# bramtoula/multi_robot_SLAM_separators

Measured on AMD Instinct MI355X. Metric: candidate keyframe-pair verifications/sec (NetVLAD NN + ORB match + RANSAC) @1/2/4/8 GPU, higher is better.
Workload: dtype u8+f16+f32+f64

## Files before the change

### multi_robot_slam_separators_amd/csrc/k_match.hip

```cpp
#include "sf_internal.hpp"
#include "sf_match_device.hpp"
#include <type_traits>

namespace {

__device__ __forceinline__ uint32_t bcnt_acc(uint32_t x, uint32_t acc) {
  uint32_t r;
  asm("v_bcnt_u32_b32 %0, %1, %2" : "=v"(r) : "v"(x), "v"(acc));
  return r;
}

template <int W, int NQ>
__device__ __forceinline__ void knn2_scan(const uint32_t* __restrict__ dF, int Kf, const uint32_t (&q)[NQ][W],
                                          uint32_t (&k1)[NQ], uint32_t (&k2)[NQ]) {
#pragma unroll 4
  for (int f = 0; f < Kf; ++f) {
    const uint32_t* r = dF + (size_t)f * W;
    uint32_t x[W];
#pragma unroll
    for (int c = 0; c < W; ++c) x[c] = r[c];
#pragma unroll
    for (int j = 0; j < NQ; ++j) {
      uint32_t d = 0;
#pragma unroll
// ... 448 lines not shown
        constexpr int JP = NTL - 1;
        float t;
        const int jp = j == 0 ? JP : j - 1;
        mf_pipe_half1(acc0, A4[0], A4[1], A4[2], A4[3], B4[j][0], B4[j][1], c0, acc1, b[jp], s[jp], t);
        mf_pipe_half2(acc0, A4[2], A4[3], B4[j][2], B4[j][3], acc1, b[jp], s[jp], t);
        mf_pipe_half1(acc1, A4[0], A4[1], A4[2], A4[3], B4[j + 1][0], B4[j + 1][1], c0, acc0, b[j], s[j], t);
        mf_pipe_half2(acc1, A4[2], A4[3], B4[j + 1][2], B4[j + 1][3], acc0, b[j], s[j], t);
      }
    }
  }
  mf_pipe_drain(acc1, b[NTL - 1], s[NTL - 1]);
}

__device__ __forceinline__ float mf_max(float a, float b) {
  float r;
  asm("v_max_f32 %0, %1, %2" : "=v"(r) : "v"(a), "v"(b));
  return r;
}
__device__ __forceinline__ float mf_min(float a, float b) {
  float r;
  asm("v_min_f32 %0, %1, %2" : "=v"(r) : "v"(a), "v"(b));
  return r;
}
__device__ __forceinline__ float mf_max3(float a, float b, float c) {
  float r;
  asm("v_max3_f32 %0, %1, %2, %3" : "=v"(r) : "v"(a), "v"(b), "v"(c));
  return r;
}

constexpr int mf_passes(int ntl) { return ntl == 1 ? 1 : ntl / 2; }

template <int W, int NTL, bool PIPE = false>
__device__ __forceinline__ void mf_scan(const uint32_t* fromD, int Kf, const MfB<W, NTL>& B, int lane,
                                        uint32_t (&d1)[mf_passes(NTL)], uint32_t (&d2)[mf_passes(NTL)],
                                        int (&idx)[mf_passes(NTL)]) {
  constexpr int KS = W / 2;
  const int r = lane & 31, h = lane >> 5;
  uint32_t m88, c22;
  asm volatile("v_mov_b32 %0, 0x88888888" : "=v"(m88));
  asm volatile("v_mov_b32 %0, 0x22222222" : "=v"(c22));
  float cin[16], b[NTL], s[NTL];
  const float hoff = h ? 4.f * MF_FR : 0.f;
#pragma unroll
  for (int i = 0; i < 16; ++i) cin[i] = -(float)((i & 3) + 8 * (i >> 2)) * MF_FR - hoff;
#pragma unroll
  for (int j = 0; j < NTL; ++j) { b[j] = -INFINITY; s[j] = -INFINITY; }
  const int n_full = Kf >> 5;
  uint32_t raw[KS];
  load_raw<KS>(fromD + (size_t)min(r, Kf - 1) * W + KS * h, raw);
  const uint32_t* nxt = fromD + (size_t)r * W + KS * h;
  if constexpr (PIPE && W == 8 && (NTL == 2 || NTL == 4)) {
    mf_scan_tiles_pipe<NTL>(fromD, n_full, Kf & 31, B, cin, b, s, m88, c22, raw, nxt);
  } else {
    for (int mt = 0; mt < n_full; ++mt) knn2_mfma_tile<W, NTL, false>(fromD, Kf, mt, r, h, B.Bf, cin, b, s, m88, c22, raw, nxt);
    if (Kf & 31) knn2_mfma_tile<W, NTL, true>(fromD, Kf, n_full, r, h, B.Bf, cin, b, s, m88, c22, raw, nxt);
  }
  const float org = (float)(32 * (((Kf + 31) >> 5) - 1)) * MF_FR;
#pragma unroll
  for (int p = 0; p < mf_passes(NTL); ++p) {
    float mb, ms, ob, os;
    int ts;
    if constexpr (NTL == 1) {
      mb = b[0]; ms = s[0]; ts = 24 * W - 2 * (int)B.psum;
      ob = __shfl_xor(mb, 32); os = __shfl_xor(ms, 32);
    } else {
      const int j0 = 2 * p, j1 = 2 * p + 1;
      mb = h ? b[j1] : b[j0]; ms = h ? s[j1] : s[j0]; ts = 24 * W - 2 * (int)((B.psum >> (16 * p + 8 * h)) & 0xFFu);
      ob = __shfl_xor(h ? b[j0] : b[j1], 32); os = __shfl_xor(h ? s[j0] : s[j1], 32);
    }
    const float nb = mf_max(mb, ob) - org;
    const float ns = mf_max3(mf_min(mb, ob), ms, os) - org;
    const float dot1 = 2.f * ceilf(nb * 0.5f), dot2 = 2.f * ceilf(ns * 0.5f);
    idx[p] = (int)((dot1 - nb) * 2048.f);
    d1[p] = (uint32_t)((32 * W - ts - (int)dot1) >> 1);
    d2[p] = ns == -INFINITY ? 0xFFFFu : (uint32_t)((32 * W - ts - (int)dot2) >> 1);
  }
}

template <int W, int NTL, bool PIPE = false>
__device__ __forceinline__ void knn2_mfma(const uint32_t* fromD, int Kf, const uint32_t* __restrict__ dT, int Kt,
                                          const int (&tile)[NTL], int lane, uint32_t (&d1)[mf_passes(NTL)],
                                          uint32_t (&d2)[mf_passes(NTL)], int (&idx)[mf_passes(NTL)]) {
  asm volatile("" : "+v"(lane));
  MfB<W, NTL> B;
  mf_load_b<W, NTL>(dT, Kt, tile, lane, B);
  mf_scan<W, NTL, PIPE>(fromD, Kf, B, lane, d1, d2, idx);
}

template <int W>
__device__ __forceinline__ uint32_t mf_repair_d2(const uint32_t* fromD, int Kf, const uint32_t* __restrict__ q_row, int idx,
                                                 uint32_t d2) {
  if ((idx & 27) == 27) return d2;
  uint32_t q[W];
  load_raw<W>(q_row, q);
  const int base = (idx & ~31) + (idx & 4);
#pragma unroll 1
  for (int g = 0; g < 32; g += 8) {
#pragma unroll
    for (int k = 0; k < 4; ++k) {
      const int row = base + g + k;
      uint32_t x[W];
      load_raw<W>(fromD + (size_t)row * W, x);
      uint32_t d = 0;
#pragma unroll
      for (int c = 0; c < W; ++c) d = bcnt_acc(x[c] ^ q[c], d);
      const bool other = row < Kf && row != idx && (g + k) != 27;
      d2 = other ? min(d2, d) : d2;
    }
  }
  return d2;
}

__device__ __forceinline__ int mf_rank_below(unsigned long long mask) {
  return (int)__builtin_amdgcn_mbcnt_hi((uint32_t)(mask >> 32), __builtin_amdgcn_mbcnt_lo((uint32_t)mask, 0u));
}

template <int W>
__device__ __forceinline__ bool mf_repair_accept(const uint32_t* fromD, int Kf, const uint32_t* __restrict__ q_row, int idx,
                                                 uint32_t d1, uint32_t d2, float nndr, bool active) {
  bool acc = false, exact = active;
  if (nndr >= 0.f) {
    if (active) {
      uint32_t pmin = d2;
      if ((idx & 27) != 27) {
        uint32_t q[4];
        load_raw<4>(q_row, q);
        const int base = (idx & ~31) + (idx & 4);
        const uint32_t ok = ((1u << min(Kf - base, 31)) - 1u) & ~(1u << (idx - base)) & ~(1u << 27);
        uint32_t no = __builtin_amdgcn_alignbit(~ok, ~ok, 23);
#pragma unroll 1
        for (int g = 0; g < 32; g += 8) {
#pragma unroll
          for (int k = 0; k < 4; ++k) {
            uint32_t x[4];
            load_raw<4>(fromD + (size_t)(base + g + k) * W, x);
            uint32_t p = no & (512u << k);
#pragma unroll
            for (int c = 0; c < 4; ++c) p = bcnt_acc(x[c] ^ q[c], p);
            pmin = min(pmin, p);
          }
          no = __builtin_amdgcn_alignbit(no, no, 8);
        }
      }
      acc = !((float)d1 > nndr * (float)pmin);
      exact = !acc;
    }
  }
  if (__ballot(exact)) {
    if (exact) acc = !((float)d1 > nndr * (float)mf_repair_d2<W>(fromD, Kf, q_row, idx, d2));
  }
  return acc;
}

template <int W, int NQ, int NT, int MF_NTL = 2, bool MF_PIPE = false>
__device__ __forceinline__ bool match_v2_body(const StoreView& st, int pair, int sF, int sT, float nndr, int min_inliers,
                                              int est, uint32_t* out, CorrHeader& hdr_out, PassState& pass_out,
                                              int32_t* __restrict__ list, int32_t* __restrict__ counter, int* smem,
                                              unsigned long long* trace_row = nullptr) {
  constexpr int NW = NT / 64;
  const int tid = threadIdx.x;
  const int lane = tid & 63, wave = __builtin_amdgcn_readfirstlane(tid >> 6);
  const int kcap = st.kcap;
  if ((unsigned)sF >= (unsigned)st.n_slots || (unsigned)sT >= (unsigned)st.n_slots) {
    if (tid == 0) {
      CorrHeader h = {0, 0, 0, 0};
      hdr_out = h;
      write_null_pass(pass_out, 0);
    }
    return false;
  }
  const int4 mF = st.meta[sF], mT = st.meta[sT];
  const int Kf = mF.x, Kt = mT.x;
  const uint32_t* dF = st.desc + (size_t)sF * kcap * W;
  const uint32_t* dT = st.desc + (size_t)sT * kcap * W;

  uint32_t* fromD = reinterpret_cast<uint32_t*>(smem);
  int* cnt = smem + kcap * W;
  int* owner = cnt + kcap;
  int* misc = owner + kcap;

  {
    const uint4* src = reinterpret_cast<const uint4*>(dF);
    uint4* dst = reinterpret_cast<uint4*>(fromD);
    for (int i = tid; i < Kf * (W / 4); i += NT) dst[i] = src[i];
  }
  for (int i = tid; i < Kf; i += NT) cnt[i] = 0;
  if (tid < 16) misc[tid] = 0;
  __syncthreads();
  SF_TRACE_ROW_MARK(trace_row, 32);

  int rejected = 0;
  if constexpr (NQ == 0) {
    if (Kf > 0) {
      constexpr int NTL = W == 8 ? MF_NTL : 1;
      const int n_nt = (Kt + 31) >> 5;
      auto group = [&](auto g, int t0) {
        constexpr int G = decltype(g)::value, NP = mf_passes(G);
        int tl[G], f[NP];
        uint32_t a1[NP], a2[NP];
#pragma unroll
        for (int j = 0; j < G; ++j) tl[j] = t0 + j * NW;
        knn2_mfma<W, G, MF_PIPE>(fromD, Kf, dT, Kt, tl, lane, a1, a2, f);
        int t[NP];
        bool on[NP], acc[NP], redo[NP];
#pragma unroll
        for (int p = 0; p < NP; ++p) {
          t[p] = G == 1 ? tl[0] * 32 + lane : (tl[2 * p] + (lane >> 5) * NW) * 32 + (lane & 31);
          on[p] = (G > 1 || lane < 32) && t[p] < Kt;
          acc[p] = (Kf >= 2) && !((float)a1[p] > nndr * (float)a2[p]);
          redo[p] = on[p] && Kf >= 2 && (acc[p] || !(nndr >= 0.f));
        }
        if constexpr (NP == 1) {
          if (__ballot(redo[0])) {
            const bool r = mf_repair_accept<W>(fromD, Kf, dT + (size_t)t[0] * W, f[0], a1[0], a2[0], nndr, redo[0]);
            acc[0] = redo[0] ? r : acc[0];
          }
        } else {
          static_assert(NP == 2, "a group has one or two decode passes");
          const unsigned long long bal0 = __ballot(redo[0]), bal1 = __ballot(redo[1]);
          const int n0 = __popcll(bal0), n1 = __popcll(bal1);
          const bool merged = nndr >= 0.f && n0 != 0 && n1 != 0 && n0 + n1 <= 64;
          int tgt = 0;
          uint32_t m0 = 0, m1 = 0;
          bool mine = false;
          if (merged) {
            const int jf = mf_rank_below(~bal0), r1 = mf_rank_below(bal1);
            const int dest = redo[0] ? 64 - n0 + lane - jf : jf;
            const int slot = __builtin_amdgcn_ds_permute(dest << 2, lane);
            tgt = __builtin_amdgcn_ds_bpermute((redo[1] ? r1 : n1 + lane - r1) << 2, slot);
            m0 = (uint32_t)__builtin_amdgcn_ds_permute(tgt << 2, (int)((uint32_t)t[1] | ((uint32_t)f[1] << 16)));
            m1 = (uint32_t)__builtin_amdgcn_ds_permute(tgt << 2, (int)(a1[1] | (a2[1] << 16)));
            mine = !redo[0] && jf < n1;
          }
#pragma unroll 1
          for (int it = 0; it < 2; ++it) {
            bool act = it ? redo[1] : redo[0];
            int wt = it ? t[1] : t[0], wf = it ? f[1] : f[0];
            uint32_t w1 = it ? a1[1] : a1[0], w2 = it ? a2[1] : a2[0];
            if (mine) {
              act = true;
              wt = (int)(m0 & 0xFFFFu); wf = (int)(m0 >> 16);
              w1 = m1 & 0xFFFFu; w2 = m1 >> 16;
            }
            if (__ballot(act)) {
              const bool r = mf_repair_accept<W>(fromD, Kf, dT + (size_t)wt * W, wf, w1, w2, nndr, act);
              if (merged) {
                const bool back = __builtin_amdgcn_ds_bpermute(tgt << 2, (int)r) != 0;
                acc[0] = redo[0] ? r : acc[0];
                acc[1] = redo[1] ? back : acc[1];
              } else if (it) {
                acc[1] = redo[1] ? r : acc[1];
              } else {
                acc[0] = redo[0] ? r : acc[0];
              }
            }
            if (merged) break;
          }
        }
#pragma unroll
        for (int p = 0; p < NP; ++p) {
          if (on[p] && acc[p]) match_claim(cnt, owner, f[p], t[p]);
          rejected += __popcll(__ballot(on[p] && !acc[p]));
        }
      };
      for (int t0 = wave; t0 < n_nt; t0 += NW * NTL) {
        const int avail = (n_nt - t0 + NW - 1) / NW;
        if constexpr (NTL >= 4) {
          if (avail >= 3) { group(std::integral_constant<int, 4>{}, t0); continue; }
        }
        if constexpr (NTL >= 2) {
          if (avail >= 2) { group(std::integral_constant<int, 2>{}, t0); continue; }
        }
        group(std::integral_constant<int, 1>{}, t0);
      }
    }
  } else if (Kf > 0) {
    for (int base = 0; base < Kt; base += NQ * NT) {

      uint32_t q[NQ][W], d1[NQ], d2[NQ], chunk[NQ];
#pragma unroll
      for (int j = 0; j < NQ; ++j) {
        const int t = base + j * NT + tid;
        load_desc<W>(dT, t, t < Kt, q[j]);
        d1[j] = 0xFFFFu;
        d2[j] = 0xFFFFu;
        chunk[j] = 0;
      }
      const int wave_rows = Kt - base - (tid & ~63);
      const int groups = wave_rows <= 0 ? 0 : min(NQ, (wave_rows + NT - 1) / NT);
      if (groups == NQ) {
        knn2_scan_lds<W, NQ>(fromD, Kf, q, d1, d2, chunk);
      } else if (groups > 0) {
#pragma unroll
        for (int j = 0; j < NQ; ++j) {
          if (j < groups) {
            uint32_t qq[1][W], a1[1] = {0xFFFFu}, a2[1] = {0xFFFFu}, ch[1] = {0};
#pragma unroll
            for (int c = 0; c < W; ++c) qq[0][c] = q[j][c];
            knn2_scan_lds<W, 1>(fromD, Kf, qq, a1, a2, ch);
            d1[j] = a1[0]; d2[j] = a2[0]; chunk[j] = ch[0];
          }
        }
      }
#pragma unroll
      for (int j = 0; j < NQ; ++j) {
        const int t = base + j * NT + tid;
        if (t < Kt) {
          const uint32_t b1 = d1[j] & 0xFFFFu, b2 = d2[j] & 0xFFFFu;
          const bool acc = (Kf >= 2) && !((float)b1 > nndr * (float)b2);
          if (acc) {
            int f = (int)chunk[j];
            const int fend = min(f + MATCH_CH, Kf);
            for (; f < fend; ++f) {
              const uint32_t* r = fromD + (size_t)f * W;
              uint32_t d = 0;
#pragma unroll
              for (int c = 0; c < W; ++c) d += __popc(r[c] ^ q[j][c]);
              if (d == b1) break;
            }
            match_claim(cnt, owner, f, t);
          } else {
            ++rejected;
          }
        }
      }
    }
  }
  if constexpr (NQ != 0) {
    for (int off = 32; off >= 1; off >>= 1) rejected += __shfl_xor(rejected, off);
  }
  if (lane == 0 && rejected) atomicAdd(&misc[0], rejected);
  SF_TRACE_ROW_MARK(trace_row, 33);
  __syncthreads();
  SF_TRACE_ROW_MARK(trace_row, 34);

  int running = 0;
  for (int base = 0; base < Kf; base += NT) {
    const int f = base + tid;
    const bool flag = (f < Kf) && (cnt[f] == 1);
    const unsigned long long bal = __ballot(flag);
    const int before = __popcll(bal & ((1ull << lane) - 1ull));
    if (lane == 0) misc[4 + wave] = __popcll(bal);
    __syncthreads();
    int woff = 0, total = 0;
#pragma unroll
    for (int w = 0; w < NW; ++w) {
      int c = misc[4 + w];
      if (w < wave) woff += c;
      total += c;
    }
    if (flag) out[running + woff + before] = (uint32_t)f | ((uint32_t)owner[f] << 16);
    running += total;
    __syncthreads();
  }
  const int n_corr = running;
  SF_TRACE_ROW_MARK(trace_row, 35);

  const MatchGates G = match_gates(Kf, Kt, mF, mT, misc[0], n_corr, min_inliers, est);
  const bool motion = G.motion, survivor = G.survivor;
  if (motion && !survivor)
    corr_count_finite<NT>(st.xyz + (size_t)sF * kcap * 3, st.xyz + (size_t)sT * kcap * 3, out, n_corr, est == 0, &misc[2]);
  if (tid == 0) {
    CorrHeader h;
    h.n_corr = n_corr;
    h.words_from = G.words_from;
    h.words_to = G.words_to;
    h.words_to_2d = G.unique_to;
    hdr_out = h;
    write_null_pass(pass_out, (motion && !survivor) ? misc[2] : 0);
    if (survivor && list) worklist_append(list, counter, pair);
  }
  return survivor;
}

template <int W, int NQ, int NT>
__global__ void __launch_bounds__(NT)
k_match_global_v2(StoreView st, const int32_t* __restrict__ pair_from, const int32_t* __restrict__ pair_to,
                  float nndr, int min_inliers, int est, uint32_t* __restrict__ corr, CorrHeader* __restrict__ hdr,
                  PassState* __restrict__ pass, int32_t* __restrict__ list, int32_t* __restrict__ counter) {
  extern __shared__ __attribute__((aligned(16))) int smem[];
  const int pair = (int)blockIdx.x;
  match_v2_body<W, NQ, NT>(st, pair, pair_from[pair], pair_to[pair], nndr, min_inliers, est, corr + (size_t)pair * st.kcap,
                           hdr[pair], pass[pair], list, counter, smem);
}

template <int W, int NT>
__global__ void __launch_bounds__(NT, 2)
k_match_global_mf(StoreView st, const int32_t* __restrict__ pair_from, const int32_t* __restrict__ pair_to,
                  float nndr, int min_inliers, int est, uint32_t* __restrict__ corr, CorrHeader* __restrict__ hdr,
                  PassState* __restrict__ pass, int32_t* __restrict__ list, int32_t* __restrict__ counter) {
  extern __shared__ __attribute__((aligned(16))) int smem[];
  const int pair = (int)blockIdx.x;
  match_v2_body<W, 0, NT, 4>(st, pair, pair_from[pair], pair_to[pair], nndr, min_inliers, est,
                             corr + (size_t)pair * st.kcap, hdr[pair], pass[pair], list, counter, smem);
}

template <int W, int NQ, int NT>
void launch_match_v2(sf_context* c, StoreView st, const int32_t* d_from, const int32_t* d_to, int n) {
  size_t lds = sf_match_lds_bytes(st.kcap, W);
  if (const char* v = getenv("SF_MATCH_LDS_PAD")) lds += (size_t)atoi(v);
  if constexpr (NQ == 0) sf_launch_pass1(c, k_match_global_mf<W, NT>, NT, lds, st, d_from, d_to, n);
  else sf_launch_pass1(c, k_match_global_v2<W, NQ, NT>, NT, lds, st, d_from, d_to, n);
}

template <int W, int NQ, int NT, bool L2 = false>
void launch_match(sf_context* c, StoreView st, const int32_t* d_from, const int32_t* d_to, int n) {
  sf_launch_pass1(c, k_match_global<W, NQ, NT, L2>, NT, (size_t)(2 * st.kcap + 16) * sizeof(int), st, d_from, d_to, n);
}

}

int sf_launch_match_global(sf_context* c, StoreView st, const int32_t* d_from, const int32_t* d_to, int n) {
  if (n <= 0) return SF_OK;
  if (c->params.desc_type == 2) return sf_launch_match_global_u8(c, st, d_from, d_to, n);
  if (c->params.desc_type == 1) {
    sf_prof_begin(c, SF_K_MATCH);
    if (st.w == 64) launch_match<64, 1, 256, true>(c, st, d_from, d_to, n);
    else launch_match<128, 1, 256, true>(c, st, d_from, d_to, n);
    sf_prof_end(c, SF_K_MATCH);
    SF_HIP(c, hipGetLastError());
    return SF_OK;
  }
  int variant = c->match_variant;
  if (variant == 0) {
    const size_t lds_v2 = sf_match_lds_bytes(st.kcap, st.w);
    variant = lds_v2 <= 64 * 1024 ? (c->match_mfma && st.kcap <= MF_MAX_ROWS ? 10256 : 12256) : 2256;
  }
  sf_prof_begin(c, SF_K_MATCH);
  switch (variant) {
    case 2256:
      if (st.w == 8) launch_match<8, 2, 256>(c, st, d_from, d_to, n);
      else launch_match<16, 2, 256>(c, st, d_from, d_to, n);
      break;
    case 10256:
      if (st.w == 8) launch_match_v2<8, 0, 256>(c, st, d_from, d_to, n);
      else launch_match_v2<16, 0, 256>(c, st, d_from, d_to, n);
      break;
    case 12256:
      if (st.w == 8) launch_match_v2<8, 2, 256>(c, st, d_from, d_to, n);
      else launch_match_v2<16, 2, 256>(c, st, d_from, d_to, n);
      break;
    default:
      sf_prof_end(c, SF_K_MATCH);
      return sf_fail(c, SF_EINVAL, "unknown match kernel variant %d", variant);
  }
  sf_prof_end(c, SF_K_MATCH);
  SF_HIP(c, hipGetLastError());
  return SF_OK;
}
```

### multi_robot_slam_separators_amd/csrc/k_verify.hip

```cpp
#ifndef SF_PNP_CHAIN_OCC
#define SF_PNP_CHAIN_OCC 3
#endif
#ifndef SF_MATCH_PIPE
#define SF_MATCH_PIPE 1
#endif
#ifndef SF_PNP_CHAIN_OCC4
#define SF_PNP_CHAIN_OCC4 2
#endif
#include "k_match.hip"
#include "k_ransac.hip"
#include "k_guided.hip"
#include "k_pnp.hip"

namespace {

struct FusedTail {
  PassState pass1, pass2;
  CorrHeader hdr1, hdr2;
  uint8_t guided_flag;
  int32_t stream_slot;
};

struct BaHandover {
  uint8_t* mask1;
  uint8_t* mask2;
  uint8_t* est2;
};

#ifndef SF_EST_CAP
#define SF_EST_CAP 256
#endif

__device__ __forceinline__ void stream_accepted(int pair, const sf_result* __restrict__ out, const DeviceParams& P,
                                                int32_t& s_slot) {
  const AcceptStream& S = P.accept;
  const int tid = (int)threadIdx.x;
  if (tid == 0) {
    const bool ok = out[pair].success != 0;
    if (S.flags) S.flags[pair] = ok ? 1 : 0;
    int slot = -1;
    if (ok) {
      const unsigned sl = atomicAdd(S.counter, 1u);
      if (sl < (unsigned)S.cap) { slot = (int)sl; S.index[sl] = pair; }
    }
    s_slot = slot;
  }
  __syncthreads();
  const int slot = s_slot;
  if (slot >= 0 && tid < (int)(sizeof(sf_result) / 16)) {
    const uint4 v = reinterpret_cast<const uint4*>(out + pair)[tid];
    reinterpret_cast<uint4*>(S.records + slot)[tid] = v;
    if (S.records2) reinterpret_cast<uint4*>(S.records2 + slot)[tid] = v;
  }
}

template <int W, int NW = 4, int PART = 0>
__device__ __forceinline__ void chain_after_match(const StoreView& st, int pair, int sF, int sT, bool est1, FusedTail& T,
                                                  uint32_t* cl, unsigned char* chain_lds, uint32_t* __restrict__ corr2,
                                                  CorrHeader* __restrict__ hdr2, PassState* __restrict__ pass1,
                                                  PassState* __restrict__ pass2, uint8_t* __restrict__ guided_flag,
                                                  sf_result* __restrict__ out, const DeviceParams& P,
                                                  const BaHandover& H) {
  constexpr int NT = 64 * NW;
  const int tid = threadIdx.x;
  const int kcap = st.kcap;
  __builtin_amdgcn_s_setprio(3);
  if constexpr (PART != 2) {
    if (est1) {
      ransac_body<0, NW>(st, pair, sF, sT, cl, T.hdr1.n_corr, T.pass1, P, chain_lds, kcap, 2,
                         PART == 1 ? H.mask1 + (size_t)pair * kcap : nullptr);
      if constexpr (PART == 0 || PART == 3) {
        if (P.force_3dof && tid == 0) pass_to3dof(T.pass1, 2);
      }
      __syncthreads();
    }
    if constexpr (PART == 1) {
      if (tid == 0) pass1[pair] = T.pass1;
      return;
    }
  }
  const bool est2 = guided_body<W, false, NW>(st, pair, sF, sT, T.pass1, T.pass2, T.guided_flag, cl, T.hdr2, nullptr, nullptr,
                                              P, reinterpret_cast<int*>(chain_lds));
  __syncthreads();
  const bool hand_over = PART == 3 && !(est2 && T.hdr2.n_corr > SF_EST_CAP);
  if (P.dbg_corr || PART == 2 || hand_over) {
    const int n = T.hdr2.n_corr;
    for (int i = tid; i < n; i += NT) corr2[(size_t)pair * kcap + i] = cl[i];
    if (tid == 0) hdr2[pair] = T.hdr2;
  }
  if constexpr (PART == 3) {
    if (tid == 0) {
      if (est1) pass1[pair] = T.pass1;
      H.est2[pair] = hand_over ? (est2 ? 1 : 0) : 2;
      if (hand_over) { pass2[pair] = T.pass2; guided_flag[pair] = T.guided_flag; }
    }
    if (hand_over) return;
  }
  if (est2) {
    ransac_body<0, NW>(st, pair, sF, sT, cl, T.hdr2.n_corr, T.pass2, P, chain_lds, kcap, 11,
                       PART == 2 ? H.mask2 + (size_t)pair * kcap : nullptr);
    if constexpr (PART == 0 || PART == 3) {
      if (P.force_3dof && tid == 0) pass_to3dof(T.pass2, 1);
    }
    __syncthreads();
  }
  SF_TRACE_MARK(P, pair, 17);
  if constexpr (PART == 2) {
    if (tid == 0) { pass2[pair] = T.pass2; guided_flag[pair] = T.guided_flag; H.est2[pair] = est2 ? 1 : 0; }
    return;
  }
  if (tid == 0) {
    if (P.dbg_corr) { pass1[pair] = T.pass1; pass2[pair] = T.pass2; guided_flag[pair] = T.guided_flag; }
    finalize_one(T.pass1, T.pass2, T.guided_flag, out[pair]);
  }
  if (P.accept_on) stream_accepted(pair, out, P, T.stream_slot);
}

template <int W, int NQ, bool WIDE = false>
__global__ void __launch_bounds__(SF_BLOCK, WIDE ? 2 : 4)
k_verify_fused(StoreView st, const int32_t* __restrict__ pair_from, const int32_t* __restrict__ pair_to,
               uint32_t* __restrict__ corr1, CorrHeader* __restrict__ hdr1, PassState* __restrict__ pass1,
               uint32_t* __restrict__ corr2, CorrHeader* __restrict__ hdr2, PassState* __restrict__ pass2,
               uint8_t* __restrict__ guided_flag, sf_result* __restrict__ out, DeviceParams P, int tail_off,
               PairSource src) {
  extern __shared__ __attribute__((aligned(16))) unsigned char smem_raw[];
  const int pair = blockIdx.x;
  const int tid = threadIdx.x;
  const int kcap = st.kcap;
  int sF, sT;
  if (src.cand) {
    sF = -1; sT = -1;
    if ((unsigned)pair < *src.count) {
      const uint2 rc = src.cand[pair];
      if ((int)rc.x < src.n_l && (int)rc.y < src.n_r) {
        const int f = src.slot_other + (int)rc.y, t = src.slot_local + (int)rc.x;
        if ((unsigned)f < (unsigned)src.n_slots && (unsigned)t < (unsigned)src.n_slots) { sF = f; sT = t; }
      }
    }
  } else {
    sF = pair_from[pair]; sT = pair_to[pair];
  }
  FusedTail& T = *reinterpret_cast<FusedTail*>(smem_raw + tail_off);
  uint32_t* cl = reinterpret_cast<uint32_t*>(smem_raw);
  unsigned char* chain_lds = smem_raw + (size_t)kcap * 4;
  SF_TRACE_MARK(P, pair, 0);
  const bool est1 = match_v2_body<W, NQ, SF_BLOCK, WIDE ? 4 : 2>(st, pair, sF, sT, P.nndr, P.min_inliers, 0, cl, T.hdr1, T.pass1,
                                                   nullptr, nullptr, reinterpret_cast<int*>(smem_raw),
                                                   P.dbg_trace ? P.dbg_trace + (size_t)pair * SF_TRACE_SLOTS : nullptr);
  __syncthreads();
  SF_TRACE_MARK(P, pair, 1);
  if (P.dbg_corr) {
    const int n = T.hdr1.n_corr;
    for (int i = tid; i < n; i += SF_BLOCK) corr1[(size_t)pair * kcap + i] = cl[i];
    if (tid == 0) hdr1[pair] = T.hdr1;
  }
  chain_after_match<W>(st, pair, sF, sT, est1, T, cl, chain_lds, corr2, hdr2, pass1, pass2, guided_flag, out, P,
                       BaHandover{nullptr, nullptr, nullptr});
}

template <int W, int NTL = 4, int MINW = 3>
__global__ void __launch_bounds__(SF_BLOCK, MINW)
k_match_split(StoreView st, const int32_t* __restrict__ pair_from, const int32_t* __restrict__ pair_to,
              uint32_t* __restrict__ corr1, CorrHeader* __restrict__ hdr1, PassState* __restrict__ pass1,
              CorrHeader* __restrict__ hdr2, PassState* __restrict__ pass2, uint8_t* __restrict__ guided_flag,
              int32_t* __restrict__ list, int32_t* __restrict__ counter, sf_result* __restrict__ out, DeviceParams P,
              int est) {
  extern __shared__ __attribute__((aligned(16))) int smem_i[];
  const int pair = blockIdx.x;
  SF_TRACE_MARK(P, pair, 0);
  const bool survivor = match_v2_body<W, 0, SF_BLOCK, NTL, SF_MATCH_PIPE != 0>(st, pair, pair_from[pair], pair_to[pair], P.nndr, P.min_inliers,
                                                         est, corr1 + (size_t)pair * st.kcap, hdr1[pair], pass1[pair],
                                                         list, counter, smem_i,
                                                         P.dbg_trace ? P.dbg_trace + (size_t)pair * SF_TRACE_SLOTS : nullptr);
  SF_TRACE_MARK(P, pair, 36);
  if (!survivor && threadIdx.x == 0) {
    const PassState p = pass1[pair];
    if (P.dbg_corr) {
      const CorrHeader h = {0, 0, 0, 0};
      hdr2[pair] = h; pass2[pair] = p; guided_flag[pair] = 0;
    }
    finalize_one(p, p, 0, out[pair]);
    if (P.accept_on && P.accept.flags) P.accept.flags[pair] = 0;
  }
}


template <int W, int NW, int PART>
__global__ void __launch_bounds__(64 * NW, 4)
k_chain(StoreView st, const int32_t* __restrict__ pair_from, const int32_t* __restrict__ pair_to,
        const uint32_t* __restrict__ corr1, const CorrHeader* __restrict__ hdr1, PassState* __restrict__ pass1,
        uint32_t* __restrict__ corr2, CorrHeader* __restrict__ hdr2, PassState* __restrict__ pass2,
        uint8_t* __restrict__ guided_flag, const int32_t* __restrict__ list, const int32_t* __restrict__ counter,
        sf_result* __restrict__ out, DeviceParams P, int tail_off, BaHandover H) {
  extern __shared__ __attribute__((aligned(16))) unsigned char smem_raw[];
  if ((int)blockIdx.x >= *counter) return;
  const int pair = list[blockIdx.x];
  const int tid = threadIdx.x;
  const int kcap = st.kcap;
  const int sF = pair_from[pair], sT = pair_to[pair];
  FusedTail& T = *reinterpret_cast<FusedTail*>(smem_raw + tail_off);
  uint32_t* cl = reinterpret_cast<uint32_t*>(smem_raw);
  unsigned char* chain_lds = smem_raw + (size_t)kcap * 4;
  bool est1 = true;
  if constexpr (PART != 2) {
    const CorrHeader h1 = hdr1[pair];
    if constexpr (PART == 3) est1 = h1.n_corr > SF_EST_CAP;
    if (tid == 0) { T.hdr1 = h1; T.pass1 = pass1[pair]; }
    if (est1)
      for (int i = tid; i < h1.n_corr; i += 64 * NW) cl[i] = corr1[(size_t)pair * kcap + i];
  } else {
    if (tid == 0) T.pass1 = pass1[pair];
  }
  __syncthreads();
  if (PART != 3 || est1) SF_TRACE_MARK(P, pair, 1);
  chain_after_match<W, NW, PART>(st, pair, sF, sT, est1, T, cl, chain_lds, corr2, hdr2, pass1, pass2, guided_flag, out, P, H);
}

template <int PASS>
__global__ void __launch_bounds__(64, 4)
k_chain_est(StoreView st, const int32_t* __restrict__ pair_from, const int32_t* __restrict__ pair_to,
            const uint32_t* __restrict__ corr, const CorrHeader* __restrict__ hdr, PassState* __restrict__ pass1,
            PassState* __restrict__ pass2, const uint8_t* __restrict__ guided_flag, const uint8_t* __restrict__ est2,
            const int32_t* __restrict__ list, const int32_t* __restrict__ counter, sf_result* __restrict__ out,
            DeviceParams P) {
  extern __shared__ __attribute__((aligned(16))) unsigned char smem_raw[];
  if ((int)blockIdx.x >= *counter) return;
  const int pair = list[blockIdx.x];
  const int run = PASS == 1 ? 1 : est2[pair];
  if (run == 2) return;
  const int n_corr = hdr[pair].n_corr;
  if (PASS == 1 && n_corr > SF_EST_CAP) return;
  __builtin_amdgcn_s_setprio(3);
  if constexpr (PASS == 1) {
    SF_TRACE_MARK(P, pair, 1);
    ransac_body<0, 1>(st, pair, pair_from[pair], pair_to[pair], corr + (size_t)pair * st.kcap, n_corr, pass1[pair], P,
                      smem_raw, SF_EST_CAP, 2);
    if (P.force_3dof && threadIdx.x == 0) pass_to3dof(pass1[pair], 2);
  } else {
    if (run) {
      ransac_body<0, 1>(st, pair, pair_from[pair], pair_to[pair], corr + (size_t)pair * st.kcap, n_corr, pass2[pair], P,
                        smem_raw, SF_EST_CAP, 11);
      if (P.force_3dof && threadIdx.x == 0) pass_to3dof(pass2[pair], 1);
    }
    SF_TRACE_MARK(P, pair, 17);
    if (threadIdx.x == 0) finalize_one(pass1[pair], pass2[pair], guided_flag[pair], out[pair]);
    if (P.accept_on) {
      __syncthreads();
      stream_accepted(pair, out, P, *reinterpret_cast<int32_t*>(smem_raw));
    }
  }
}

template <int W, int NQ, bool WIDE = false>
int launch_fused(sf_context* c, StoreView st, const int32_t* d_from, const int32_t* d_to, int n, sf_result* d_out,
                 size_t lds, int tail_off) {
  const Workspace& w = *c->w;
  const int rc = sf_dyn_lds(c, k_verify_fused<W, NQ, WIDE>, lds);
  if (rc != SF_OK) return rc;
  hipLaunchKernelGGL((k_verify_fused<W, NQ, WIDE>), dim3(n), dim3(SF_BLOCK), lds, c->stream, st, d_from, d_to, w.corr(1),
                     w.hdr(1), w.pass(1), w.corr(2), w.hdr(2), w.pass(2), w.guided_flags(), d_out, c->dparams, tail_off,
                     c->pair_src);
  return SF_OK;
}

size_t fused_tail_offset(const sf_context* c, const StoreView& st, bool with_match = true) {
  const int nc = c->dparams.grid_gx * c->dparams.grid_gy;
  const size_t match = with_match ? sf_match_lds_bytes(st.kcap, st.w) : 0;
  const size_t guided = (size_t)st.kcap * 4 + sf_guided_lds_bytes(st.kcap, nc);
  const size_t ransac = (size_t)st.kcap * 4 + ((sf_ransac_lds_bytes(st.kcap, c->dparams.iterations) + 15) & ~(size_t)15);
  return (std::max(match, std::max(guided, ransac)) + 15) & ~(size_t)15;
}

}

size_t sf_fused_lds_bytes(const sf_context* c, const StoreView& st) {
  if (!c->fused || c->dparams.estimation_type != 0 || c->dparams.bidirectional) return 0;
  if (c->params.desc_type != 0) return 0;
  const size_t match = sf_match_lds_bytes(st.kcap, st.w);
  if (match > 64 * 1024 || c->match_variant != 0) return 0;
  const size_t lds = fused_tail_offset(c, st) + ((sizeof(FusedTail) + 15) & ~(size_t)15);
  return lds <= 160 * 1024 ? lds : 0;
}

int sf_launch_verify_fused(sf_context* c, StoreView st, const int32_t* d_from, const int32_t* d_to, int n,
                           sf_result* d_out) {
  if (n <= 0) return SF_OK;
  const size_t lds = sf_fused_lds_bytes(c, st);
  if (lds == 0 || c->dparams.bundle_adjustment) return sf_fail(c, SF_EINVAL, "fused verification pipeline not applicable");
  const int tail_off = (int)fused_tail_offset(c, st);
  int rc;
  sf_prof_begin(c, SF_K_FUSED);
  const bool mf = c->match_mfma && st.kcap <= MF_MAX_ROWS;
  static const bool wide_off = getenv("SF_FUSED_WIDE_OFF") != nullptr;
  static const bool wide_all = getenv("SF_FUSED_WIDE_ALL") != nullptr;
  if (mf && st.w == 8 && (lds * 4 > 160 * 1024 || wide_all) && !wide_off)
    rc = launch_fused<8, 0, true>(c, st, d_from, d_to, n, d_out, lds, tail_off);
  else if (mf) rc = st.w == 8 ? launch_fused<8, 0>(c, st, d_from, d_to, n, d_out, lds, tail_off)
                              : launch_fused<16, 0>(c, st, d_from, d_to, n, d_out, lds, tail_off);
  else rc = st.w == 8 ? launch_fused<8, 2>(c, st, d_from, d_to, n, d_out, lds, tail_off)
                      : launch_fused<16, 2>(c, st, d_from, d_to, n, d_out, lds, tail_off);
  sf_prof_end(c, SF_K_FUSED);
  if (rc != SF_OK) return rc;
  SF_HIP(c, hipGetLastError());
  return SF_OK;
}

namespace {

template <int W, int PART, int NW>
__global__ void __launch_bounds__(64 * NW, NW == 4 ? SF_PNP_CHAIN_OCC4 : SF_PNP_CHAIN_OCC)
k_chain_pnp(StoreView st, const int32_t* __restrict__ pair_from, const int32_t* __restrict__ pair_to,
            const uint32_t* __restrict__ corr1, const CorrHeader* __restrict__ hdr1, PassState* __restrict__ pass1,
            uint32_t* __restrict__ corr2, CorrHeader* __restrict__ hdr2, PassState* __restrict__ pass2,
            uint8_t* __restrict__ guided_flag, const int32_t* __restrict__ list, const int32_t* __restrict__ counter,
            sf_result* __restrict__ out, DeviceParams P, BaHandover H) {
  extern __shared__ __attribute__((aligned(16))) unsigned char smem_raw[];
  if ((int)blockIdx.x >= *counter) return;
  const int pair = list[blockIdx.x];
  const int sF = pair_from[pair], sT = pair_to[pair];
  const int kcap = st.kcap;
  __builtin_amdgcn_s_setprio(3);
  SF_TRACE_MARK(P, pair, 1);
  if constexpr (PART != 2) {
    pnp_body<0, NW>(st, pair, pair_from, pair_to, corr1, hdr1, pass1, P, smem_raw, 37,
                    PART == 1 ? H.mask1 + (size_t)pair * kcap : nullptr);
    if constexpr (PART == 1) return;
    if (P.force_3dof && threadIdx.x == 0) pass_to3dof(pass1[pair], 2);
    __syncthreads();
  }
  const bool est2 = guided_body<W, false, NW>(st, pair, sF, sT, pass1[pair], pass2[pair], guided_flag[pair],
                                              corr2 + (size_t)pair * kcap, hdr2[pair], nullptr, nullptr, P,
                                              reinterpret_cast<int*>(smem_raw));
  __syncthreads();
  SF_TRACE_MARK(P, pair, 42);
  if (est2) {
// ... 361 lines not shown
```

### multi_robot_slam_separators_amd/csrc/sf_match_device.hpp

```cpp
#pragma once
#include "sf_device_math.hpp"
#include "sf_internal.hpp"

__device__ __forceinline__ void write_null_pass(PassState& out, int matches) {
  PassState ps;
#pragma unroll
  for (int i = 0; i < 12; ++i) ps.T[i] = 0.f;
  ps.var = 1.0; ps.var_ang = 1.0;
  ps.is_null = 1;
  ps.inliers = 0;
  ps.matches = matches;
  ps.pad = 0;
  out = ps;
}

__device__ inline void pass_to3dof(PassState& ps, int times) {
  if (ps.is_null) return;
  for (int t = 0; t < times; ++t) sfd::to3dof_canon(ps.T);
}

__device__ inline void merge_backward_pose(PassState& a, const PassState& b) {
  if (b.is_null) return;
  float inv[12];
  sfd::rigid_inverse_canon(b.T, inv);
  if (a.is_null) {
#pragma unroll
    for (int i = 0; i < 12; ++i) a.T[i] = inv[i];
    a.is_null = 0;
    a.var = b.var;
    a.var_ang = b.var_ang;
  } else {
    float mid[12];
    sfd::interpolate_half_canon(a.T, inv, mid);
#pragma unroll
    for (int i = 0; i < 12; ++i) a.T[i] = mid[i];
    a.var = (a.var + b.var) / 2.0;
    a.var_ang = (a.var_ang + b.var_ang) / 2.0;
  }
}

template <int NW, class ToOf>
__device__ __forceinline__ int corr_compact(int Kf, uint32_t* out, int* misc, ToOf to_of) {
  constexpr int NT = 64 * NW;
  const int tid = (int)threadIdx.x;
  const int lane = tid & 63, wave = tid >> 6;
  int running = 0;
  for (int base = 0; base < Kf; base += NT) {
    const int i = base + tid;
    const int m = (i < Kf) ? to_of(i) : -1;
    const bool flag = m >= 0;
    const unsigned long long bal = __ballot(flag);
    const int before = __popcll(bal & ((1ull << lane) - 1ull));
    if (lane == 0) misc[4 + wave] = __popcll(bal);
    __syncthreads();
    int woff = 0, total = 0;
#pragma unroll
    for (int w = 0; w < NW; ++w) {
      int c = misc[4 + w];
      if (w < wave) woff += c;
      total += c;
    }
    if (flag) out[running + woff + before] = (uint32_t)i | ((uint32_t)m << 16);
    running += total;
    __syncthreads();
  }
  return running;
}

template <int NT>
__device__ __forceinline__ void corr_count_finite(const float* xF, const float* xT, const uint32_t* out, int n_corr,
                                                  bool with_to, int* count) {
  for (int i = (int)threadIdx.x; i < n_corr; i += NT) {
    uint32_t c = out[i];
    const float* a = xF + 3 * (c & 0xFFFFu);
    const float* b = xT + 3 * (c >> 16);
    bool ok = isfinite(a[0]) && isfinite(a[1]) && isfinite(a[2]);
    if (with_to)
      ok = ok && isfinite(b[0]) && isfinite(b[1]) && isfinite(b[2]) && (a[0] != 0.f || a[1] != 0.f || a[2] != 0.f) &&
           (b[0] != 0.f || b[1] != 0.f || b[2] != 0.f);
    if (ok) atomicAdd(count, 1);
  }
  __syncthreads();
}

__device__ __forceinline__ void worklist_append(int32_t* __restrict__ list, int32_t* __restrict__ counter, int pair) {
  int pos = atomicAdd(counter, 1);
  list[pos] = pair;
}


__device__ __forceinline__ void match_claim(int* cnt, int* owner, int f, int t) {
  atomicAdd(&cnt[f], 1);
  owner[f] = t;
}

struct MatchGates {
  int unique_to, words_from, words_to;
  bool motion, survivor;
};
__device__ __forceinline__ MatchGates match_gates(int Kf, int Kt, const int4& mF, const int4& mT, int rejected_to, int n_corr,
                                                  int min_inliers, int est) {
  MatchGates g;
  g.unique_to = (Kf > 0 && Kt > 0) ? rejected_to + n_corr : 0;
  g.words_from = (Kf > 0 && mF.y > 0) ? Kf : 0;
  g.words_to = (mT.y > 0) ? g.unique_to : 0;
  const int unique_to = g.unique_to, words_from = g.words_from, words_to = g.words_to;
  g.motion = est == 0 ? (unique_to > 0 && words_from >= min_inliers && words_to >= min_inliers)
           : est == 1 ? (unique_to > 0 && words_from >= min_inliers && unique_to >= min_inliers)
                      : (est == 3 && unique_to > 0 && ((words_from >= min_inliers && unique_to >= min_inliers) ||
                                                       (words_to >= min_inliers && Kf >= min_inliers)));
  g.survivor = est == 3 ? (g.motion && n_corr > 0) : (g.motion && n_corr >= min_inliers && n_corr >= (est == 0 ? 3 : 4));
  return g;
}

struct MatchPair {
  int sF, sT;
  int4 mF, mT;
  int* cnt;
  int* owner;
  int* misc;
};

__device__ __forceinline__ bool match_slot_outside(const StoreView& st, int sF, int sT) {
  return (unsigned)sF >= (unsigned)st.n_slots || (unsigned)sT >= (unsigned)st.n_slots;
}
__device__ __forceinline__ void match_report_outside(CorrHeader& hdr_out, PassState& pass_out) {
  if (threadIdx.x == 0) {
    CorrHeader h = {0, 0, 0, 0};
    hdr_out = h;
    write_null_pass(pass_out, 0);
  }
}

template <int NT>
__device__ __forceinline__ void match_begin(const StoreView& st, int sF, int sT, int* book, MatchPair& M) {
  M.sF = sF; M.sT = sT;
  M.mF = st.meta[sF]; M.mT = st.meta[sT];
  M.cnt = book;
  M.owner = book + st.kcap;
  M.misc = book + 2 * st.kcap;
  const int tid = threadIdx.x;
  for (int i = tid; i < M.mF.x; i += NT) M.cnt[i] = 0;
  if (tid < 16) M.misc[tid] = 0;
}

template <int NT>
__device__ __forceinline__ void match_finish(const StoreView& st, int pair, const MatchPair& M, int min_inliers, int est,
                                             int rejected, uint32_t* out, CorrHeader& hdr_out, PassState& pass_out,
                                             int32_t* __restrict__ list, int32_t* __restrict__ counter) {
  const int tid = threadIdx.x;
  const int kcap = st.kcap;
  const int Kf = M.mF.x, Kt = M.mT.x;
  int* cnt = M.cnt;
  int* owner = M.owner;
  int* misc = M.misc;
  for (int off = 32; off >= 1; off >>= 1) rejected += __shfl_xor(rejected, off);
  if ((tid & 63) == 0 && rejected) atomicAdd(&misc[0], rejected);
  __syncthreads();

  const int n_corr = corr_compact<NT / 64>(Kf, out, misc, [&](int f) { return cnt[f] == 1 ? owner[f] : -1; });
  const MatchGates G = match_gates(Kf, Kt, M.mF, M.mT, misc[0], n_corr, min_inliers, est);
// ... 14 lines not shown
```

Measured before the change: 26.68 million.

## Add lean match path with batched descriptor staging, single-barrier compaction, parallel null result write

Adds a LEAN variant of the match body used by k_match_split. It stages the from-descriptors into LDS four loads at a time, with the cnt zeroing folded into the same loop. It replaces the per-tile barrier compaction with a single ballot pass that packs per-wave counts as bytes, so only one barrier is needed. Non-surviving pairs now have their sf_result written in parallel 16-byte chunks by 23 threads, instead of thread 0 reading the pass back and calling finalize_one. The risks are register pressure from the extra arrays and reliance on a hard-coded sf_result layout, which the static_assert checks.

```diff
diff --git a/multi_robot_slam_separators_amd/csrc/k_match.hip b/multi_robot_slam_separators_amd/csrc/k_match.hip
--- a/multi_robot_slam_separators_amd/csrc/k_match.hip
+++ b/multi_robot_slam_separators_amd/csrc/k_match.hip
@@ -624,11 +624,11 @@
   return acc;
 }
 
-template <int W, int NQ, int NT, int MF_NTL = 2, bool MF_PIPE = false>
+template <int W, int NQ, int NT, int MF_NTL = 2, bool MF_PIPE = false, bool LEAN = false>
 __device__ __forceinline__ bool match_v2_body(const StoreView& st, int pair, int sF, int sT, float nndr, int min_inliers,
                                               int est, uint32_t* out, CorrHeader& hdr_out, PassState& pass_out,
                                               int32_t* __restrict__ list, int32_t* __restrict__ counter, int* smem,
-                                              unsigned long long* trace_row = nullptr) {
+                                              unsigned long long* trace_row = nullptr, int* null_matches = nullptr) {
   constexpr int NW = NT / 64;
   const int tid = threadIdx.x;
   const int lane = tid & 63, wave = __builtin_amdgcn_readfirstlane(tid >> 6);
@@ -639,6 +639,7 @@
       hdr_out = h;
       write_null_pass(pass_out, 0);
     }
+    if constexpr (LEAN) *null_matches = 0;
     return false;
   }
   const int4 mF = st.meta[sF], mT = st.meta[sT];
@@ -651,12 +652,29 @@
   int* owner = cnt + kcap;
   int* misc = owner + kcap;
 
-  {
+  if constexpr (LEAN) {
+    const int n16 = Kf * (W / 4);
+    const uint4* src = reinterpret_cast<const uint4*>(dF);
+    uint4* dst = reinterpret_cast<uint4*>(fromD);
+    for (int i = tid; i < n16; i += 4 * NT) {
+      uint4 v[4];
+#pragma unroll
+      for (int u = 0; u < 4; ++u)
+        v[u] = *reinterpret_cast<const uint4*>(reinterpret_cast<const char*>(src) + (uint32_t)min(i + u * NT, n16 - 1) * 16u);
+      asm volatile("" ::"v"(v[0].x), "v"(v[0].y), "v"(v[0].z), "v"(v[0].w), "v"(v[1].x), "v"(v[1].y), "v"(v[1].z), "v"(v[1].w),
+                   "v"(v[2].x), "v"(v[2].y), "v"(v[2].z), "v"(v[2].w), "v"(v[3].x), "v"(v[3].y), "v"(v[3].z), "v"(v[3].w));
+#pragma unroll
+      for (int u = 0; u < 4; ++u) {
+        if (i + u * NT < n16) dst[i + u * NT] = v[u];
+        if (i + u * NT < Kf) cnt[i + u * NT] = 0;
+      }
+    }
+  } else {
     const uint4* src = reinterpret_cast<const uint4*>(dF);
     uint4* dst = reinterpret_cast<uint4*>(fromD);
     for (int i = tid; i < Kf * (W / 4); i += NT) dst[i] = src[i];
-  }
-  for (int i = tid; i < Kf; i += NT) cnt[i] = 0;
+    for (int i = tid; i < Kf; i += NT) cnt[i] = 0;
+  }
   if (tid < 16) misc[tid] = 0;
   __syncthreads();
   SF_TRACE_ROW_MARK(trace_row, 32);
@@ -807,6 +825,45 @@
   SF_TRACE_ROW_MARK(trace_row, 34);
 
   int running = 0;
+  if constexpr (LEAN) {
+    constexpr int MAXT = MF_MAX_ROWS / NT;
+    static_assert(MAXT <= 8 && NW <= 4, "two words of byte counts per wavefront in misc[4..12)");
+    const int ntrip = (Kf + NT - 1) / NT;
+    unsigned long long bal[MAXT];
+    uint32_t pk[2] = {0u, 0u};
+#pragma unroll
+    for (int t = 0; t < MAXT; ++t) bal[t] = 0ull;
+#pragma unroll
+    for (int t = 0; t < MAXT; ++t) {
+      if (t >= ntrip) break;
+      const int f = t * NT + tid;
+      bal[t] = __ballot((f < Kf) && (cnt[f] == 1));
+      pk[t >> 2] |= (uint32_t)__popcll(bal[t]) << (8 * (t & 3));
+    }
+    if (lane == 0) { misc[4 + 2 * wave] = (int)pk[0]; misc[5 + 2 * wave] = (int)pk[1]; }
+    __syncthreads();
+    uint32_t tot[2][2] = {{0u, 0u}, {0u, 0u}}, mine[2][2] = {{0u, 0u}, {0u, 0u}};
+#pragma unroll
+    for (int w = 0; w < NW; ++w) {
+#pragma unroll
+      for (int j = 0; j < 2; ++j) {
+        if (j == 1 && ntrip <= 4) continue;
+        const uint32_t x = (uint32_t)__builtin_amdgcn_readfirstlane(misc[4 + 2 * w + j]);
+        const uint32_t e = x & 0x00FF00FFu, o = (x >> 8) & 0x00FF00FFu;
+        tot[j][0] += e; tot[j][1] += o;
+        if (w < wave) { mine[j][0] += e; mine[j][1] += o; }
+      }
+    }
+#pragma unroll
+    for (int t = 0; t < MAXT; ++t) {
+      if (t >= ntrip) break;
+      const int sh = 16 * ((t & 3) >> 1);
+      const int total = (int)((tot[t >> 2][t & 1] >> sh) & 0xFFFFu), woff = (int)((mine[t >> 2][t & 1] >> sh) & 0xFFFFu);
+      const int f = t * NT + tid;
+      if (__builtin_amdgcn_inverse_ballot_w64(bal[t])) out[running + woff + mf_rank_below(bal[t])] = (uint32_t)f | ((uint32_t)owner[f] << 16);
+      running += total;
+    }
+  } else
   for (int base = 0; base < Kf; base += NT) {
     const int f = base + tid;
     const bool flag = (f < Kf) && (cnt[f] == 1);
@@ -830,8 +887,10 @@
 
   const MatchGates G = match_gates(Kf, Kt, mF, mT, misc[0], n_corr, min_inliers, est);
   const bool motion = G.motion, survivor = G.survivor;
-  if (motion && !survivor)
+  if (motion && !survivor) {
+    if constexpr (LEAN) __syncthreads();
     corr_count_finite<NT>(st.xyz + (size_t)sF * kcap * 3, st.xyz + (size_t)sT * kcap * 3, out, n_corr, est == 0, &misc[2]);
+  }
   if (tid == 0) {
     CorrHeader h;
     h.n_corr = n_corr;
@@ -842,6 +901,7 @@
     write_null_pass(pass_out, (motion && !survivor) ? misc[2] : 0);
     if (survivor && list) worklist_append(list, counter, pair);
   }
+  if constexpr (LEAN) *null_matches = (motion && !survivor) ? misc[2] : 0;
   return survivor;
 }
 
diff --git a/multi_robot_slam_separators_amd/csrc/k_verify.hip b/multi_robot_slam_separators_amd/csrc/k_verify.hip
--- a/multi_robot_slam_separators_amd/csrc/k_verify.hip
+++ b/multi_robot_slam_separators_amd/csrc/k_verify.hip
@@ -158,6 +158,25 @@
                        BaHandover{nullptr, nullptr, nullptr});
 }
 
+__device__ __forceinline__ void write_null_result(sf_result& out, int matches) {
+  static_assert(sizeof(sf_result) == 23 * 16 && offsetof(sf_result, covariance) == 56 && offsetof(sf_result, inliers) == 344 &&
+                offsetof(sf_result, matches) == 348 && offsetof(sf_result, inliers_pass1) == 352 &&
+                offsetof(sf_result, matches_pass1) == 356 && offsetof(sf_result, success) == 360,
+                "the 16-byte chunks below follow sf_result's layout");
+  const int c = (int)threadIdx.x;
+  if (c >= 23) return;
+  constexpr double D = SF_NULL_VAR <= 1e-9 ? 1e-9 : SF_NULL_VAR;
+  const unsigned long long d = (unsigned long long)__double_as_longlong(D);
+  const uint32_t dlo = (uint32_t)d, dhi = (uint32_t)(d >> 32);
+  const bool up = c == 3 || c == 10 || c == 17, low = c == 7 || c == 14 || c == 21;
+  uint4 v;
+  v.x = low ? dlo : 0u;
+  v.y = low ? dhi : (c == 22 ? (uint32_t)matches : 0u);
+  v.z = up ? dlo : 0u;
+  v.w = up ? dhi : (c == 21 ? (uint32_t)matches : 0u);
+  reinterpret_cast<uint4*>(&out)[c] = v;
+}
+
 template <int W, int NTL = 4, int MINW = 3>
 __global__ void __launch_bounds__(SF_BLOCK, MINW)
 k_match_split(StoreView st, const int32_t* __restrict__ pair_from, const int32_t* __restrict__ pair_to,
@@ -168,19 +187,22 @@
   extern __shared__ __attribute__((aligned(16))) int smem_i[];
   const int pair = blockIdx.x;
   SF_TRACE_MARK(P, pair, 0);
-  const bool survivor = match_v2_body<W, 0, SF_BLOCK, NTL, SF_MATCH_PIPE != 0>(st, pair, pair_from[pair], pair_to[pair], P.nndr, P.min_inliers,
+  int matches = 0;
+  const bool survivor = match_v2_body<W, 0, SF_BLOCK, NTL, SF_MATCH_PIPE != 0, true>(st, pair, pair_from[pair], pair_to[pair], P.nndr, P.min_inliers,
                                                          est, corr1 + (size_t)pair * st.kcap, hdr1[pair], pass1[pair],
                                                          list, counter, smem_i,
-                                                         P.dbg_trace ? P.dbg_trace + (size_t)pair * SF_TRACE_SLOTS : nullptr);
+                                                         P.dbg_trace ? P.dbg_trace + (size_t)pair * SF_TRACE_SLOTS : nullptr,
+                                                         &matches);
   SF_TRACE_MARK(P, pair, 36);
-  if (!survivor && threadIdx.x == 0) {
-    const PassState p = pass1[pair];
-    if (P.dbg_corr) {
-      const CorrHeader h = {0, 0, 0, 0};
-      hdr2[pair] = h; pass2[pair] = p; guided_flag[pair] = 0;
-    }
-    finalize_one(p, p, 0, out[pair]);
-    if (P.accept_on && P.accept.flags) P.accept.flags[pair] = 0;
+  if (!survivor) {
+    write_null_result(out[pair], matches);
+    if (threadIdx.x == 0) {
+      if (P.dbg_corr) {
+        const CorrHeader h = {0, 0, 0, 0};
+        hdr2[pair] = h; write_null_pass(pass2[pair], matches); guided_flag[pair] = 0;
+      }
+      if (P.accept_on && P.accept.flags) P.accept.flags[pair] = 0;
+    }
   }
 }
 
diff --git a/multi_robot_slam_separators_amd/csrc/sf_match_device.hpp b/multi_robot_slam_separators_amd/csrc/sf_match_device.hpp
--- a/multi_robot_slam_separators_amd/csrc/sf_match_device.hpp
+++ b/multi_robot_slam_separators_amd/csrc/sf_match_device.hpp
@@ -2,11 +2,12 @@
 #include "sf_device_math.hpp"
 #include "sf_internal.hpp"
 
+constexpr double SF_NULL_VAR = 1.0;
 __device__ __forceinline__ void write_null_pass(PassState& out, int matches) {
   PassState ps;
 #pragma unroll
   for (int i = 0; i < 12; ++i) ps.T[i] = 0.f;
-  ps.var = 1.0; ps.var_ang = 1.0;
+  ps.var = SF_NULL_VAR; ps.var_ang = SF_NULL_VAR;
   ps.is_null = 1;
   ps.inliers = 0;
   ps.matches = matches;
```

Result: faster. 27.24 million, median of 6 (+2.1%).
